# DJNing/articulated-object-nerf

Hardware: AMD Instinct MI355X
Metric: rays/sec at 640×480×(64c+128f) samples; PSNR vs reference (higher is better)
Workload: dtype f16x3 (fp16 hi/lo split MFMA, fp32 accumulate)

## Files before the change

### articulated-object-nerf_amd/aonerf/_lib.py

```python
import ctypes
import os

import torch

_HERE = os.path.dirname(os.path.abspath(__file__))
LIB_PATH = os.path.join(os.path.dirname(_HERE), "lib", "libaonerf.so")

c_i64, c_int, c_float, c_size, vp = ctypes.c_int64, ctypes.c_int, ctypes.c_float, ctypes.c_size_t, ctypes.c_void_p

PREC = {"fp32": 0, "f16x3": 1}
PREC_F16X3_TRAIN = 4
PREC_BF16 = 2
ACT_NONE, ACT_VANILLA, ACT_ARTIC = 0, 1, 2
OPACITY = {None: 0, "mse": 1, "ce": 2, "autorf": 3}


class AonMlpParams(ctypes.Structure):
    _fields_ = [("pts_w", vp * 8), ("pts_b", vp * 8), ("density_w", vp), ("density_b", vp),
                ("bottleneck_w", vp), ("bottleneck_b", vp), ("views_w", vp), ("views_b", vp),
                ("rgb_w", vp), ("rgb_b", vp), ("w_rows", c_i64 * 12), ("w_cols", c_i64 * 12),
                ("b_len", c_i64 * 12)]


class AonMlpArtParams(ctypes.Structure):
# ... 113 lines not shown
    "aon_sample_along_rays": (c_int, [vp, vp, c_i64, c_int, vp, vp, vp, vp, vp, vp]),
    "aon_pos_enc": (c_int, [vp, c_i64, c_int, c_int, vp, vp]),
    "aon_sample_rays": (c_int, [vp, vp, c_int, c_i64, c_int, c_int, c_float, vp, c_i64, c_int,
                                c_float, vp, vp, vp, vp, vp]),
    "aon_cast_rays": (c_int, [vp, vp, vp, c_i64, c_int, vp, c_i64, vp, c_int, c_int, vp, vp]),
    "aon_cast_rays_tiled": (c_int, [vp, vp, vp, c_i64, c_int, c_int, c_int, c_int, vp, vp]),
    "aon_sample_pdf": (c_int, [vp, c_i64, vp, c_i64, c_i64, c_int, c_int, vp, c_i64, vp, c_int,
                               vp, vp, vp, vp, vp]),
    "aon_composite_march": (c_int, [vp, vp, vp, c_i64, c_int, c_int, c_int, vp, c_i64, c_int, vp,
                                    vp, vp, vp, vp, vp]),
    "aon_mlp_packed_bytes": (c_size, [c_int]),
    "aon_mlp_read_status": (c_int, [vp, c_size, ctypes.POINTER(ctypes.c_uint32), vp]),
    "aon_mlp_pack": (c_int, [ctypes.POINTER(AonMlpParams), c_int, vp, vp]),
    "aon_mlp_fwd": (c_int, [vp, c_int, vp, vp, vp, vp, c_i64, c_int, c_int, vp, vp]),
    "aon_mlp_fwd_encoded": (c_int, [vp, c_int, vp, vp, c_i64, c_int, c_int, vp, vp]),
    "aon_mlp_fwd_train": (c_int, [vp, vp, vp, vp, vp, c_i64, c_int, vp, vp, vp, vp, vp, vp, vp]),
    "aon_mlp_fwd_train_bf16": (c_int, [vp, vp, vp, vp, vp, c_i64, c_int, vp, vp, vp, vp, vp, vp,
                                       vp, vp]),
    "aon_mlp_bwd_pack_bf16": (c_int, [ctypes.POINTER(AonMlpParams), vp, vp]),
    "aon_mlp_bwd_bf16": (c_int, [vp, vp, vp, c_i64, vp, vp, vp, vp, vp]),
    "aon_relu_masks": (c_int, [vp, c_i64, c_int, vp, vp]),
    "aon_absmax": (c_int, [vp, c_i64, vp, vp]),
    "aon_mlp_bwd_packed_bytes": (c_size, []),
    "aon_mlp_bwd_pack": (c_int, [ctypes.POINTER(AonMlpParams), vp, vp]),
    "aon_mlp_bwd": (c_int, [vp, vp, vp, c_i64, vp, vp, vp, vp, vp]),
    "aon_mlp_art_packed_bytes": (c_size, []),
    "aon_mlp_art_pack": (c_int, [ctypes.POINTER(AonMlpArtParams), vp, vp]),
    "aon_mlp_art_fwd": (c_int, [vp, vp, vp, vp, vp, c_i64, c_int, c_int, vp, vp]),
    "aon_mlp_art_fwd_points": (c_int, [vp, vp, vp, c_i64, c_int, c_int, vp, vp]),
    "aon_mlp_art_bwd_packed_bytes": (c_size, []),
# ... 195 lines not shown
```

### articulated-object-nerf_amd/aonerf/model.py

```python
import warnings

import torch
import torch.nn as nn
import torch.nn.init as init

from . import _lib as L
from . import helper
from .numerics import resolve as _resolve_numerics

_DEFAULT_GEOMETRY = dict(min_deg_point=0, max_deg_point=10, deg_view=4, netdepth=8, netwidth=256,
                         netdepth_condition=1, netwidth_condition=128, skip_layer=4, input_ch=3,
                         input_ch_view=3, num_rgb_channels=3, num_density_channels=1)


class NeRFMLP(nn.Module):

    def __init__(self, min_deg_point, max_deg_point, deg_view, netdepth: int = 8,
                 netwidth: int = 256, netdepth_condition: int = 1, netwidth_condition: int = 128,
                 skip_layer: int = 4, input_ch: int = 3, input_ch_view: int = 3,
                 num_rgb_channels: int = 3, num_density_channels: int = 1,
                 precision: str = "f16x3"):
        super().__init__()
        self.min_deg_point, self.max_deg_point, self.deg_view = min_deg_point, max_deg_point, deg_view
        self.netdepth, self.netwidth, self.skip_layer = netdepth, netwidth, skip_layer
# ... 45 lines not shown
        params = [p for m in self._layers() for p in (m.weight, m.bias)]
        L.require_gpu(*params)
        key = (self.precision,) + tuple((p.data_ptr(), p._version) for p in params)
        if key != self._packed_key:
            params = [L.contig(p.detach()) for p in params]
            prm = L.mlp_params(zip(params[0::2], params[1::2]))
            prec = L.PREC[self.precision]
            nbytes = L.lib().aon_mlp_packed_bytes(prec)
            if nbytes == 0:
                raise NotImplementedError(f"precision {self.precision!r} is not built yet")
            buf = torch.empty(nbytes // 4, dtype=torch.float32, device=params[0].device)
            L.call("aon_mlp_pack", L.ctypes.byref(prm), prec, L.ptr(buf), L.stream(buf.device))
            self._packed, self._packed_key = buf, key
        return self._packed

    def forward_rays(self, rays_o, rays_d, viewdirs, t_vals, act=L.ACT_NONE):
        L.require_gpu(rays_o, rays_d, viewdirs, t_vals)
        B, S = t_vals.shape
        raw = torch.empty((B * S, 4), device=t_vals.device)
        L.call("aon_mlp_fwd", L.ptr(self.packed_weights()), L.PREC[self.precision],
               L.ptr(L.contig(rays_o)), L.ptr(L.contig(rays_d)), L.ptr(L.contig(viewdirs)),
               L.ptr(L.contig(t_vals)), B, S, act, L.ptr(raw), L.stream(t_vals.device))
        return raw

    def forward(self, x, condition):
        L.require_gpu(x, condition)
        B, S, C = x.shape
        if C != 63 or tuple(condition.shape) != (B, 27):
            raise ValueError("NeRFMLP.forward expects x (B, S, 63) and condition (B, 27)")
        raw = torch.empty((B * S, 4), device=x.device)
        L.call("aon_mlp_fwd_encoded", L.ptr(self.packed_weights()), L.PREC[self.precision],
               L.ptr(L.contig(x)), L.ptr(L.contig(condition)), B, S, L.ACT_NONE, L.ptr(raw),
               L.stream(x.device))
        raw = raw.view(B, S, 4)
        return raw[..., :3], raw[..., 3:]


# ... 68 lines not shown
        self.fused_march, self.range_check = bool(fused_march), bool(range_check)
        self.num_levels, self.min_deg_point, self.max_deg_point = num_levels, min_deg_point, max_deg_point
        self.deg_view, self.num_coarse_samples, self.num_fine_samples = deg_view, num_coarse_samples, num_fine_samples
        self.use_viewdirs, self.noise_std, self.lindisp = use_viewdirs, noise_std, lindisp
        self.coarse_mlp = NeRFMLP(min_deg_point, max_deg_point, deg_view, precision=precision)
        self.fine_mlp = NeRFMLP(min_deg_point, max_deg_point, deg_view, precision=precision)

    def set_precision(self, precision):
        for m in (self.coarse_mlp, self.fine_mlp):
            if precision not in L.PREC:
                raise ValueError(precision)
            m.precision = precision
        return self

    def forward(self, rays, randomized, white_bkgd, near, far, *, u_coarse=None, u_fine=None,
                return_weights=False, return_intermediates=False, timers=None):
        o, d, v = rays["rays_o"], rays["rays_d"], rays["viewdirs"]
        L.require_gpu(o, d, v)
        o, d, v = L.contig(o), L.contig(d), L.contig(v)
        training = torch.is_grad_enabled() and any(p.requires_grad for p in self.parameters())
        B = o.shape[0]
        dev = o.device
        rng = torch.cuda.get_rng_state(dev) if randomized and not training else None
        ret = []
        t_vals = weights = t_next = None
        token, joined = None, {}
        cfg = self.train_numerics
        if training:
            from . import train
            if cfg.overlap_dweight and cfg.fused_backward and timers is None:
                token = train.JoinToken()
                ps = [p for m in (self.coarse_mlp, self.fine_mlp) for l in m._layers()
                      for p in (l.weight, l.bias)]
                joined = dict(zip(map(id, ps), train.Join.apply(token, *ps)))
        for level in range(2):
            with torch.no_grad():
                t_vals = t_next if t_next is not None else self._level_t(
# ... 9 lines not shown
                params = [joined.get(id(p), p) for p in params]
                comp, acc, depth, weights = RenderLevel.apply(o, d, v, t_vals, bool(white_bkgd),
                                                              noise, token, cfg, timers, *params)
                out = (comp, acc, depth, weights) if return_weights else (comp, acc, depth)
                if return_intermediates:
                    out = out + (dict(t_vals=t_vals, weights=weights),)
                ret.append(out)
                continue
            keep_w = level == 0 or return_weights or return_intermediates
            march = level == 0 and march_ok(S, self.num_fine_samples, self.fused_march)
            if march:
                keep_w = return_weights or return_intermediates
            with torch.no_grad():
                out, weights, t_next = self._render_level_fused(
                    mlp, o, d, v, t_vals, randomized, white_bkgd, level, timers, keep_w,
                    march_u=(lambda: fine_uniforms(B, self.num_fine_samples, randomized, dev,
                                                   u_fine)) if march else None)
            if not return_weights:
                out = out[:3] + out[4:]
            if not return_intermediates:
                out = out[:4] if return_weights else out[:3]
            ret.append(out)
        if (not training and self.range_check and self.coarse_mlp.precision.startswith("f16x3")
                and not torch.cuda.is_current_stream_capturing()
                and L.range_overflow([self.coarse_mlp._packed, self.fine_mlp._packed])):
            warnings.warn("NeRF: an MLP activation exceeded the fp16x3 range; re-rendered with "
                          "precision='fp32'", RuntimeWarning)
            prec = self.coarse_mlp.precision
            self.set_precision("fp32")
            if rng is not None:
                torch.cuda.set_rng_state(rng, dev)
            try:
                return self.forward(rays, randomized, white_bkgd, near, far, u_coarse=u_coarse,
                                    u_fine=u_fine, return_weights=return_weights,
                                    return_intermediates=return_intermediates, timers=timers)
            finally:
                self.set_precision(prec)
        return ret

    def _level_t(self, level, o, d, t_prev, w_prev, randomized, near, far, u_coarse, u_fine):
        return level_t_vals(level, o, d, t_prev, w_prev, randomized, near, far,
                            self.num_coarse_samples, self.num_fine_samples, self.lindisp,
                            u_coarse, u_fine)

    def _render_level_fused(self, mlp, o, d, v, t_vals, randomized, white_bkgd, level, timers,
                            keep_weights=True, march_u=None):
        B, S = t_vals.shape
        dev = o.device
        noisy = self.noise_std > 0 and randomized
        ev = _events(timers)
        raw = mlp.forward_rays(o, d, v, t_vals, act=L.ACT_NONE if noisy else L.ACT_VANILLA)
        _record(timers, ev, f"mlp{level}", B * S)
        if noisy:
            raw[:, 3] += torch.rand_like(raw[:, 3]) * self.noise_std
        act = L.ACT_VANILLA if noisy else L.ACT_NONE
        t_next = None
        ev = _events(timers)
        if march_u is not None:
            u, u_stride = march_u()
            (comp, acc, depth, weights), t_next = composite_march(
                raw, t_vals, d, white_bkgd, act, u, u_stride, self.num_fine_samples, keep_weights)
            _record(timers, ev, f"march{level}", B * S)
        else:
            comp = torch.empty((B, 3), device=dev)
            acc = torch.empty((B,), device=dev)
            weights = torch.empty((B, S), device=dev) if keep_weights else None
# ... 7 lines not shown
```

### articulated-object-nerf_amd/aonerf/render.py

```python
import math
from collections import defaultdict

import numpy as np
import torch

from . import interface
from .ray_utils import frame_rays

DEFAULT_CHUNK = 1 << 21


def _chunks(B, chunk):
    chunk = max(int(chunk or DEFAULT_CHUNK), 1)
    for i in range(0, B, chunk):
        yield i, min(i + chunk, B)


@torch.no_grad()
def render_rays(model, batch, chunk, white_bkgd, near, far):
    B = batch["rays_o"].shape[0]
    ret = defaultdict(list)
    for i, j in _chunks(B, chunk):
        sub = {k: batch[k][i:j] for k in ("rays_o", "rays_d", "viewdirs")}
        fine = model(sub, False, white_bkgd, near, far)[1]
        ret["comp_rgb"].append(fine[0])
        ret["acc"].append(fine[1])
        ret["depth"].append(fine[2])
    out = {k: torch.cat(v, 0) for k, v in ret.items()}
    if "target" in batch:
        out["psnr"] = interface.psnr_legacy(out["comp_rgb"], batch["target"]).mean()
    return out


@torch.no_grad()
def render_rays_test(model, batch, chunk, white_bkgd, near, far):
    out = render_rays(model, {k: v for k, v in batch.items() if k != "target"}, chunk, white_bkgd,
                      near, far)
    test_output = {"rgb": out["comp_rgb"]}
    for k in ("target", "instance_mask"):
        if k in batch:
            test_output[k] = batch[k]
    return test_output


@torch.no_grad()
def render_frame(model, c2w, H, W, focal, near=2.0, far=6.0, white_bkgd=True, p0=0, n=None,
                 chunk=None, timers=None):
    n = H * W - p0 if n is None else n
    rays = frame_rays(c2w, H, W, focal, p0, n)
    out = torch.empty((n, 5), device=rays["rays_o"].device)
    for i, j in _chunks(n, chunk):
        sub = {k: v[i:j] for k, v in rays.items()}
        fine = model(sub, False, white_bkgd, near, far, timers=timers)[1]
        out[i:j, 0:3] = fine[0]
        out[i:j, 3] = fine[2]
        out[i:j, 4] = fine[1]
    return out


def create_spheric_poses(radius=4.0, n=40, phi=-30.0):

    def trans_t(t):
        return np.array([[1, 0, 0, 0], [0, 1, 0, 0], [0, 0, 1, t], [0, 0, 0, 1]], np.float32)

    def rot_phi(p):
        c, s = np.cos(p), np.sin(p)
        return np.array([[1, 0, 0, 0], [0, c, -s, 0], [0, s, c, 0], [0, 0, 0, 1]], np.float32)

# ... 17 lines not shown
```

### articulated-object-nerf_amd/csrc/mlp.hip

```cpp
#include "aon_common.hpp"
#include "mlp_layout.hpp"
#include "mlp_pipe.hpp"
#include "param_check.hpp"

namespace aon {
namespace mlp {

constexpr int kWaves = 8;
constexpr int kThreads = 64 * kWaves;
constexpr int kRowsPerWave = 16;
constexpr int kRowsPerBlock = kRowsPerWave * kWaves;

__device__ __forceinline__ f4 mfma(float a, float b, f4 c) {
  return __builtin_amdgcn_mfma_f32_16x16x4f32(a, b, c, 0, 0, 0);
}

template <int LAYER, int NA, int NB, int NACC>
__device__ __forceinline__ void gemm(Pipe<kThreads>& p, const f4 (&xa)[NA], const f4 (&xb)[NB],
                                     f4 (&acc)[NACC]) {
  constexpr LayerDesc d = kLayers[LAYER];
  constexpr int U = d.u;
  static_assert(U % 4 == 0 && U <= NACC && d.ka <= NA && d.kb <= NB, "layer/array mismatch");
#pragma unroll
  for (int t = 0; t < d.ka + d.kb; ++t) {
// ... 293 lines not shown
}

extern "C" int aon_mlp_fwd(const void* packed, int precision, const float* rays_o,
                           const float* rays_d, const float* viewdirs, const float* t, int64_t B,
                           int S, int act, float* raw, aon_stream_t stream) {
  AON_REQUIRE(viewdirs && t, "null pointer");
  return mlp_launch(0, packed, precision, rays_o, rays_d, viewdirs, t, B, S, act, raw, stream);
}

extern "C" int aon_mlp_fwd_encoded(const void* packed, int precision, const float* x,
                                   const float* condition, int64_t B, int S, int act,
                                   float* raw, aon_stream_t stream) {
  return mlp_launch(1, packed, precision, x, condition, nullptr, nullptr, B, S, act, raw, stream);
}

extern "C" int aon_mlp_fwd_train(const void* packed, const float* rays_o, const float* rays_d,
                                 const float* viewdirs, const float* t, int64_t B, int S,
                                 const float* noise, float* h, float* bot, float* hv, float* raw,
                                 uint32_t* masks, aon_stream_t stream) {
  AON_REQUIRE(packed && rays_o && rays_d && viewdirs && t && h && bot && hv && raw && masks,
              "null pointer");
  AON_REQUIRE(aligned16(masks), "masks must be 16-byte aligned");
  AON_REQUIRE(B >= 0 && S >= 1, "bad shape");
  AON_REQUIRE(aligned16(packed) && aligned16(raw) && aligned16(h) && aligned16(bot) && aligned16(hv),
              "packed / output buffers must be 16-byte aligned");
  const int64_t N = B * S;
  if (N == 0) return 0;
  AON_REQUIRE((N + 127) / 128 < (1ll << 31), "too many rows");
  const TrainStore ts{h, bot, hv, noise, reinterpret_cast<uint2*>(masks)};
  return launch_f16x3(2, 1, packed, rays_o, rays_d, viewdirs, t, B, S, AON_ACT_NONE, raw,
// ... 24 lines not shown
```

### articulated-object-nerf_amd/csrc/mlp_f16x3.hip

```cpp
#include "mlp_f16x3_core.hpp"

namespace aon {
namespace mlp {

#ifndef AON_STASH_REGS
#define AON_STASH_REGS 0
#endif

#ifndef AON_STAGGER
#define AON_STAGGER 0
#endif

template <bool BF>
__host__ __device__ constexpr int stash_per() { return BF ? 3 : 6; }
template <bool BF>
__device__ __forceinline__ int enc_slot(int c, int k, int lo) { return BF ? 3 * c + k : 6 * c + 2 * k + lo; }
template <bool BF>
__device__ __forceinline__ int venc_slot(int c, int lo) { return BF ? 3 * c + 2 : 6 * c + 4 + lo; }

template <typename Net, int NCOL, bool STORE, typename T, typename FP>
__device__ __forceinline__ void vanilla_layers(FP& fp, Frag<2, NCOL>& enc, Frag<1, NCOL>& venc,
                                               Frag<8, NCOL>& x, Frag<8, NCOL>& y, f4* stash,
                                               float* bias_s, int g, int wave,
                                               const int64_t (&rows)[NCOL], int64_t N, int act,
                                               float* __restrict__ raw, const TrainStore& ts) {
  constexpr bool BF = std::is_same<T, __bf16>::value;
  fp.start();
#if AON_PRIO_HALF
  if (wave >= GeomH<NCOL>::kWaves / 2) __builtin_amdgcn_s_setprio(AON_PRIO_HALF);
#endif
  lds_float* bias_l = opaque_lds(bias_s + 4 * g);

  Frag<1, NCOL> none;
  using SP = StorePick<STORE, NCOL, T>;
  T* const th = reinterpret_cast<T*>(ts.h);
  T* const tbot = reinterpret_cast<T*>(ts.bot);
  T* const thv = reinterpret_cast<T*>(ts.hv);
  const int64_t hs = act_rows(N) * 256;
  const int64_t ms = act_rows(N) * 4;
  layer_h<Net, L0, true>(fp, none, enc, x, bias_l, g, SP::make(th, 256, rows, N, g, ts.masks));
  layer_h<Net, L1, true>(fp, x, none, y, bias_l, g, SP::make(th + 1 * hs, 256, rows, N, g, ts.masks + 1 * ms));
  layer_h<Net, L2, true>(fp, y, none, x, bias_l, g, SP::make(th + 2 * hs, 256, rows, N, g, ts.masks + 2 * ms));
  layer_h<Net, L3, true>(fp, x, none, y, bias_l, g, SP::make(th + 3 * hs, 256, rows, N, g, ts.masks + 3 * ms));
  layer_h<Net, L4, true>(fp, y, none, x, bias_l, g, SP::make(th + 4 * hs, 256, rows, N, g, ts.masks + 4 * ms));
#pragma unroll
  for (int c = 0; c < NCOL && !AON_STASH_REGS; ++c)
#pragma unroll
    for (int k = 0; k < 2; ++k) {
      enc.hi[k][c] = __builtin_bit_cast(h8, stash[64 * enc_slot<BF>(c, k, 0)]);
      if (!BF) enc.lo[k][c] = __builtin_bit_cast(h8, stash[64 * enc_slot<BF>(c, k, 1)]);
    }
  layer_h<Net, L5, true>(fp, x, enc, y, bias_l, g, SP::make(th + 5 * hs, 256, rows, N, g, ts.masks + 5 * ms));
  layer_h<Net, L6, true>(fp, y, none, x, bias_l, g, SP::make(th + 6 * hs, 256, rows, N, g, ts.masks + 6 * ms));
  layer_h<Net, L7, true>(fp, x, none, y, bias_l, g, SP::make(th + 7 * hs, 256, rows, N, g, ts.masks + 7 * ms));
  f4 dens[NCOL], rgb[NCOL];
  head_h<Net, LDEN>(fp, y, dens, bias_l, g);
  constexpr bool FOLD = std::is_same<Net, NetVanillaFoldH>::value;
  static_assert(!FOLD || !STORE, "the training forwards keep the bottleneck activation");
  if constexpr (!FOLD)
    layer_h<Net, LBOT, false>(fp, y, none, x, bias_l, g, SP::make(tbot, 256, rows, N, g));
#pragma unroll
  for (int c = 0; c < NCOL && !AON_STASH_REGS; ++c) {
    venc.hi[0][c] = __builtin_bit_cast(h8, stash[64 * venc_slot<BF>(c, 0)]);
    if (!BF) venc.lo[0][c] = __builtin_bit_cast(h8, stash[64 * venc_slot<BF>(c, 1)]);
  }
  if constexpr (FOLD) {
    layer_h<Net, LF_VIEW, true>(fp, y, venc, x, bias_l, g);
    head_h<Net, LF_RGB>(fp, x, rgb, bias_l, g);
  } else {
    layer_h<Net, LVIEW, true>(fp, x, venc, y, bias_l, g, SP::make(thv, 128, rows, N, g, ts.masks + 8 * ms));
    head_h<Net, LRGB>(fp, y, rgb, bias_l, g);
  }

  if (g == 0) {
#pragma unroll
    for (int c = 0; c < NCOL; ++c) {
      if (rows[c] < N) {
        const float s = AON_F16X3_V2 ? 1.0f : 1.0f / kActScale;
        float sig = dens[c][0] * s;
        if (STORE && ts.noise) sig = __fadd_rn(sig, ts.noise[rows[c]]);
        const f4 o = {act_rgb(rgb[c][0] * s, act), act_rgb(rgb[c][1] * s, act),
                      act_rgb(rgb[c][2] * s, act), act_sigma(sig, act)};
#ifdef AON_ABL_NO_RAW_STORE
        if (__builtin_isnan(o[0] + o[1] + o[2] + o[3]))
#endif
        *reinterpret_cast<f4*>(raw + 4 * rows[c]) = o;
      }
    }
  }
}

template <int MODE, int NCOL, bool STORE = false, bool BF = false, typename Net = NetVanillaH>
__global__ __launch_bounds__((GeomH<NCOL, BF>::kThreads), (GeomH<NCOL, BF>::kWavesPerSimd)) void k_mlp_fwd_f16x3(
    const f4* __restrict__ wstream, const float* __restrict__ bias_g, const float* __restrict__ in0,
    const float* __restrict__ in1, const float* __restrict__ in2, const float* __restrict__ in3,
    int64_t B, int S, int act, float* __restrict__ raw, TrainStore ts = {}) {
  using G = GeomH<NCOL, BF>;
  constexpr int kPer = stash_per<BF>() * NCOL;
  constexpr int kStash = AON_STASH_REGS ? 0 : G::kWaves * 64 * kPer;
  static_assert((kLdsWeights + Net::kBiasFloats / 4 + kStash) * 16 <= 160 * 1024, "LDS");
  __shared__ f4 smem[kLdsWeights + Net::kBiasFloats / 4 + kStash];
  float* bias_s = reinterpret_cast<float*>(smem + kLdsWeights);
  f4* stash = smem + kLdsWeights + Net::kBiasFloats / 4 + (threadIdx.x >> 6) * 64 * kPer +
              (threadIdx.x & 63);

  const int tid = threadIdx.x, lane = tid & 63, wave = tid >> 6;
  const int g = lane >> 4, j = lane & 15;
  const int64_t N = B * S;

  WeightPipeP<Net, G::kThreads, BF> p;
  p.wbuf = smem;
  p.src = wstream;
  p.tid = tid;
  p.lane = lane;
  p.start();
  for (int i = tid; i < Net::kBiasFloats; i += G::kThreads) bias_s[i] = bias_g[i];

  Frag<2, NCOL> enc;
  Frag<1, NCOL> venc;
  int64_t rows[NCOL];
#pragma unroll
  for (int c = 0; c < NCOL; ++c) {
    const int64_t row = (int64_t)blockIdx.x * G::kRowsPerBlock + wave * G::kRowsPerWave + 16 * c + j;
    rows[c] = row;
    const int64_t rr = row < N ? row : N - 1;
    const int64_t ray = rr / S;
    float ev[2][8], vv[8];
    if (MODE == 0) {
      const float* ro = in0 + 3 * ray;
      const float* rd = in1 + 3 * ray;
      const float* vd = in2 + 3 * ray;
      const float tt = in3[rr];
      const float x0 = __fadd_rn(ro[0], __fmul_rn(tt, rd[0]));
      const float x1 = __fadd_rn(ro[1], __fmul_rn(tt, rd[1]));
      const float x2 = __fadd_rn(ro[2], __fmul_rn(tt, rd[2]));
      const float v0 = vd[0], v1 = vd[1], v2 = vd[2];
      auto encode = [&](auto fast) {
#pragma unroll
        for (int k = 0; k < 2; ++k)
#pragma unroll
          for (int e = 0; e < 8; ++e)
          {
            ev[k][e] = pos_enc_feature_fast(x0, x1, x2, 32 * k + 8 * g + e, 0, 10, fast.value);
            __builtin_amdgcn_sched_barrier(0);
          }
#pragma unroll
        for (int e = 0; e < 8; ++e) {
          vv[e] = pos_enc_feature_fast(v0, v1, v2, 8 * g + e, 0, 4, fast.value);
          __builtin_amdgcn_sched_barrier(0);
        }
      };
      if (pos_enc_fast_ok(x0, x1, x2, 10) && pos_enc_fast_ok(v0, v1, v2, 4))
        encode(std::true_type{});
      else
        encode(std::false_type{});
    } else {
      const float* x = in0 + rr * 63;
      const float* cd = in1 + ray * 27;
#pragma unroll
      for (int k = 0; k < 2; ++k)
#pragma unroll
        for (int e = 0; e < 8; ++e) {
          const int f = 32 * k + 8 * g + e;
          ev[k][e] = f < 63 ? x[f] : 0.f;
        }
#pragma unroll
      for (int e = 0; e < 8; ++e) {
        const int f = 8 * g + e;
        vv[e] = f < 27 ? cd[f] : 0.f;
      }
    }
    if (STORE && BF && ts.enc_bf && keep_row(rows[c], N)) store_enc_bf(ts.enc_bf, rows[c], g, ev);
#pragma unroll
    for (int k = 0; k < 2; ++k) {
#pragma unroll
      for (int e = 0; e < 8; ++e) ev[k][e] *= act_scale<BF>();
      split8<BF>(ev[k], enc.hi[k][c], enc.lo[k][c], enc.ovf);
    }
#pragma unroll
    for (int e = 0; e < 8; ++e) vv[e] *= act_scale<BF>();
    split8<BF>(vv, venc.hi[0][c], venc.lo[0][c], venc.ovf);
  }

#pragma unroll
  for (int c = 0; c < NCOL && !AON_STASH_REGS; ++c) {
#pragma unroll
    for (int k = 0; k < 2; ++k) {
      stash[64 * enc_slot<BF>(c, k, 0)] = __builtin_bit_cast(f4, enc.hi[k][c]);
      if (!BF) stash[64 * enc_slot<BF>(c, k, 1)] = __builtin_bit_cast(f4, enc.lo[k][c]);
    }
    stash[64 * venc_slot<BF>(c, 0)] = __builtin_bit_cast(f4, venc.hi[0][c]);
    if (!BF) stash[64 * venc_slot<BF>(c, 1)] = __builtin_bit_cast(f4, venc.lo[0][c]);
  }

  Frag<8, NCOL> x, y;
  using WP = WeightPipeP<Net, G::kThreads, BF>;
  using T = typename std::conditional<BF, __bf16, float>::type;
  if (AON_STAGGER && NCOL == 1 && !STORE && __builtin_amdgcn_readfirstlane(wave) >= G::kWaves / 2) {
    FragPipe<WP, AON_PREFETCH, 4, BF> fp(p);
    vanilla_layers<Net, NCOL, STORE, T>(fp, enc, venc, x, y, stash, bias_s, g, wave, rows, N, act, raw, ts);
  } else {
    FragPipe<WP, AON_PREFETCH, 0, BF> fp(p);
    vanilla_layers<Net, NCOL, STORE, T>(fp, enc, venc, x, y, stash, bias_s, g, wave, rows, N, act, raw, ts);
  }
  range_report(bias_g + Net::kBiasFloats, ovf_of(x) | ovf_of(y) | enc.ovf | venc.ovf);
}

__global__ void k_pack_h(PackArgsH a, float* __restrict__ out_f) {
  const int64_t nhalf = (int64_t)a.stream_blocks * 512;
  _Float16* out = reinterpret_cast<_Float16*>(out_f);
  float* bias_out = out_f + (int64_t)a.stream_blocks * 256;
  const int64_t total = nhalf + a.bias_floats;
  const LayerDesc& last = a.layers[a.n_layers - 1];
  const int used_blocks = last.blk0 + (last.ka + last.kb) * last.u * 2;
  const StreamMap map{a.bf16, a.mx_lo, a.mx_hi};
  if (a.bf16 == 1 && !a.f16w && blockIdx.x == 0 && threadIdx.x < kStatusBytes / 4)
    reinterpret_cast<uint32_t*>(bias_out + a.bias_floats)[threadIdx.x] = 0u;
  for (int64_t e = blockIdx.x * (int64_t)blockDim.x + threadIdx.x; e < total;
       e += (int64_t)gridDim.x * blockDim.x) {
    if (e < nhalf) {
// ... 149 lines not shown
                         static_cast<int>((N + GB::kRowsPerBlock - 1) / GB::kRowsPerBlock),
                         GB::kThreads, 0, stream, ws, bias, a0, a1, a2, a3, B, S, act, raw, *ts);
    } else
      hipLaunchKernelGGL((k_mlp_fwd_f16x3<0, 1, true>), grid, GeomH<1>::kThreads, 0, stream, ws,
                         bias, a0, a1, a2, a3, B, S, act, raw, *ts);
    return launch_status("aon_mlp_fwd_train");
  }
  if (mode == 0 && ncol == 1) AON_LAUNCH_H(0, 1);
  else if (mode == 0) AON_LAUNCH_H(0, 2);
  else if (ncol == 1) AON_LAUNCH_H(1, 1);
  else AON_LAUNCH_H(1, 2);
#undef AON_LAUNCH_H
  return launch_status("aon_mlp_fwd");
}

}
}
```

### articulated-object-nerf_amd/csrc/mlp_layout.hpp

```cpp
#pragma once

namespace aon {
namespace mlp {

struct LayerDesc {
  int ka, kb;
  int u;
  int len_a, len_b;
  int out_real;
  int blk0;
  int bias0;
};

enum { L0 = 0, L1, L2, L3, L4, L5, L6, L7, LDEN, LBOT, LVIEW, LRGB, kNumLayers };

constexpr int kChunk = 16;

constexpr LayerDesc kLayers[kNumLayers] = {
    {4, 0, 16, 63, 0, 256, 0, 0},
    {16, 0, 16, 256, 0, 256, 64, 256},
    {16, 0, 16, 256, 0, 256, 320, 512},
    {16, 0, 16, 256, 0, 256, 576, 768},
    {16, 0, 16, 256, 0, 256, 832, 1024},
    {16, 4, 16, 256, 63, 256, 1088, 1280},
// ... 188 lines not shown
static_assert(NetVanillaFoldH::ok(), "inconsistent folded vanilla fp16x3 layout");
constexpr bool layout_fold_ok() {
  for (int i = 0; i < kNumLayersFold; ++i) {
    const LayerDesc& f = kLayersHFold[i];
    const LayerDesc& h = kLayersH[i < LBOT ? i : i + 1];
    if (f.ka != h.ka || f.kb != h.kb || f.u != h.u || f.len_a != h.len_a || f.len_b != h.len_b ||
        f.out_real != h.out_real)
      return false;
    if (i < LBOT && (f.blk0 != h.blk0 || f.bias0 != h.bias0)) return false;
  }
  const LayerDesc& b = kLayersH[LBOT];
  return kLayersHFold[LF_VIEW].len_a == b.out_real && kBlocksFold == kBlocks - b.ka * b.u * 2 &&
         kBiasFloatsFold == kBiasFloats - b.u * 16;
}
static_assert(layout_fold_ok(), "folded layout must be kLayersH without the bottleneck");
static_assert(NetArtH::ok(), "inconsistent articulated fp16x3 layout");
static_assert(NetBwdH::ok(), "inconsistent backward-chain fp16x3 layout");
static_assert(NetArtBwdH::ok(), "inconsistent articulated backward-chain fp16x3 layout");

struct PackArgs {
  const float* w[kNumLayers];
  const float* b[kNumLayers];
  LayerDesc layers[kNumLayers];
};

constexpr int kMaxLayersH = 24;
struct PackArgsH {
  const float* w[kMaxLayersH];
  const float* w2[kMaxLayersH];
  const float* b[kMaxLayersH];
// ... 65 lines not shown
  float* hv;
  float* enc;
  float* xyz;
  const float* noise;
  uint2* masks;
  __bf16* enc_bf;
};

int pack_f16x3(const PackArgs& a, void* packed, hipStream_t stream, bool bf16 = false,
               bool fold = false);
int pack_h(PackArgsH a, void* packed, hipStream_t stream);
int absmax(const float* x, int64_t n, uint32_t* out, hipStream_t stream);
int launch_f16x3(int mode, int ncol, const void* packed, const float* a0, const float* a1,
                 const float* a2, const float* a3, int64_t B, int S, int act, float* raw,
                 hipStream_t stream, const TrainStore* ts = nullptr);
#ifndef AON_DATAFLOW_WS_BUILD
#define AON_DATAFLOW_WS_BUILD 0
#endif
int launch_ws_f16x3(const void* packed, const float* a0, const float* a1, const float* a2,
                    const float* a3, int64_t B, int S, int act, float* raw, hipStream_t stream);
int launch_art_ws_f16x3(const void* packed, const float* a0, const float* a1, const float* a2,
                        const float* a3, int64_t B, int S, int act, float* raw, hipStream_t stream);

}
}
```

### include/aonerf.h

```cpp
#ifndef AONERF_H
#define AONERF_H

#include <stddef.h>
#include <stdint.h>

#ifdef __cplusplus
extern "C" {
#endif

typedef void* aon_stream_t;

#define AON_ABI_VERSION 13

#define AON_PREC_FP32 0
#define AON_PREC_F16X3 1
#define AON_PREC_F16X3_TRAIN 4
#define AON_PREC_BF16 2

#define AON_ACT_NONE 0
#define AON_ACT_VANILLA 1
#define AON_ACT_ARTIC 2

int aon_abi_version(void);
const char* aon_last_error(void);
// ... 53 lines not shown
size_t aon_mlp_packed_bytes(int precision);
int aon_mlp_pack(const aon_mlp_params* params, int precision, void* packed,
                 aon_stream_t stream);

int aon_mlp_read_status(const void* packed, size_t packed_bytes, uint32_t* status,
                        aon_stream_t stream);

int aon_mlp_fwd(const void* packed, int precision, const float* rays_o, const float* rays_d,
                const float* viewdirs, const float* t, int64_t B, int S, int act, float* out,
                aon_stream_t stream);


int aon_mlp_fwd_encoded(const void* packed, int precision, const float* x,
                        const float* condition, int64_t B, int S, int act, float* out,
                        aon_stream_t stream);

int aon_mlp_fwd_train(const void* packed, const float* rays_o, const float* rays_d,
                      const float* viewdirs, const float* t, int64_t B, int S, const float* noise,
                      float* h, float* bot, float* hv, float* raw, uint32_t* masks,
                      aon_stream_t stream);

int aon_mlp_fwd_train_bf16(const void* packed, const float* rays_o, const float* rays_d,
                           const float* viewdirs, const float* t, int64_t B, int S,
                           const float* noise, uint16_t* h, uint16_t* bot, uint16_t* hv,
                           float* raw, uint32_t* masks, uint16_t* enc, aon_stream_t stream);

int aon_relu_masks(const float* h, int64_t N, int width, uint32_t* masks, aon_stream_t stream);

int aon_absmax(const float* x, int64_t n, uint32_t* out, aon_stream_t stream);

// ... 171 lines not shown
```

Baseline: 1.653 million.

## Skip coarse-level RGB head in render path and precompute view encoding per ray

Adds a density-only MLP kernel that streams only the prefix of the folded weight stream up to the density head, and uses it for the coarse level when only fine outputs are requested. The fine level uses a new MODE 2 kernel that takes a per-ray precomputed view-direction encoding instead of recomputing it per sample. The render entry points now pass fine_only=True. The coarse RGB is discarded anyway, so this is meant to cut the view and RGB layers and the smaller LDS stash from the coarse pass. The cost is extra kernel variants and a per-ray pos_enc launch.

Measured after the change: 1.717 million, median of 6. 1.04x the previous value.

```diff
diff --git a/articulated-object-nerf_amd/aonerf/_lib.py b/articulated-object-nerf_amd/aonerf/_lib.py
--- a/articulated-object-nerf_amd/aonerf/_lib.py
+++ b/articulated-object-nerf_amd/aonerf/_lib.py
@@ -151,6 +151,8 @@
     "aon_mlp_pack": (c_int, [ctypes.POINTER(AonMlpParams), c_int, vp, vp]),
     "aon_mlp_fwd": (c_int, [vp, c_int, vp, vp, vp, vp, c_i64, c_int, c_int, vp, vp]),
     "aon_mlp_fwd_encoded": (c_int, [vp, c_int, vp, vp, c_i64, c_int, c_int, vp, vp]),
+    "aon_mlp_fwd_sigma": (c_int, [vp, c_int, vp, vp, vp, c_i64, c_int, c_int, vp, vp]),
+    "aon_mlp_fwd_cond": (c_int, [vp, c_int, vp, vp, vp, vp, c_i64, c_int, c_int, vp, vp]),
     "aon_mlp_fwd_train": (c_int, [vp, vp, vp, vp, vp, c_i64, c_int, vp, vp, vp, vp, vp, vp, vp]),
     "aon_mlp_fwd_train_bf16": (c_int, [vp, vp, vp, vp, vp, c_i64, c_int, vp, vp, vp, vp, vp, vp,
                                        vp, vp]),
diff --git a/articulated-object-nerf_amd/aonerf/model.py b/articulated-object-nerf_amd/aonerf/model.py
--- a/articulated-object-nerf_amd/aonerf/model.py
+++ b/articulated-object-nerf_amd/aonerf/model.py
@@ -83,13 +83,29 @@
             self._packed, self._packed_key = buf, key
         return self._packed
 
-    def forward_rays(self, rays_o, rays_d, viewdirs, t_vals, act=L.ACT_NONE):
-        L.require_gpu(rays_o, rays_d, viewdirs, t_vals)
+    def forward_rays(self, rays_o, rays_d, viewdirs, t_vals, act=L.ACT_NONE, cond=None):
+        L.require_gpu(rays_o, rays_d, viewdirs, t_vals, cond)
         B, S = t_vals.shape
         raw = torch.empty((B * S, 4), device=t_vals.device)
+        if cond is not None:
+            if tuple(cond.shape) != (B, 27):
+                raise ValueError("forward_rays expects cond (B, 27)")
+            L.call("aon_mlp_fwd_cond", L.ptr(self.packed_weights()), L.PREC[self.precision],
+                   L.ptr(L.contig(rays_o)), L.ptr(L.contig(rays_d)), L.ptr(L.contig(cond)),
+                   L.ptr(L.contig(t_vals)), B, S, act, L.ptr(raw), L.stream(t_vals.device))
+            return raw
         L.call("aon_mlp_fwd", L.ptr(self.packed_weights()), L.PREC[self.precision],
                L.ptr(L.contig(rays_o)), L.ptr(L.contig(rays_d)), L.ptr(L.contig(viewdirs)),
                L.ptr(L.contig(t_vals)), B, S, act, L.ptr(raw), L.stream(t_vals.device))
+        return raw
+
+    def forward_sigma(self, rays_o, rays_d, t_vals, act=L.ACT_NONE):
+        L.require_gpu(rays_o, rays_d, t_vals)
+        B, S = t_vals.shape
+        raw = torch.empty((B * S, 4), device=t_vals.device)
+        L.call("aon_mlp_fwd_sigma", L.ptr(self.packed_weights()), L.PREC[self.precision],
+               L.ptr(L.contig(rays_o)), L.ptr(L.contig(rays_d)), L.ptr(L.contig(t_vals)), B, S, act,
+               L.ptr(raw), L.stream(t_vals.device))
         return raw
 
     def forward(self, x, condition):
@@ -188,13 +204,16 @@
         return self
 
     def forward(self, rays, randomized, white_bkgd, near, far, *, u_coarse=None, u_fine=None,
-                return_weights=False, return_intermediates=False, timers=None):
+                return_weights=False, return_intermediates=False, timers=None, fine_only=False):
         o, d, v = rays["rays_o"], rays["rays_d"], rays["viewdirs"]
         L.require_gpu(o, d, v)
         o, d, v = L.contig(o), L.contig(d), L.contig(v)
         training = torch.is_grad_enabled() and any(p.requires_grad for p in self.parameters())
         B = o.shape[0]
         dev = o.device
+        fine_only = bool(fine_only) and not (training or return_weights or return_intermediates)
+        two_pass = fine_only and self.coarse_mlp.precision == self.fine_mlp.precision == "f16x3"
+        cond = helper.pos_enc(v, 0, self.deg_view) if two_pass else None
         rng = torch.cuda.get_rng_state(dev) if randomized and not training else None
         ret = []
         t_vals = weights = t_next = None
@@ -234,13 +253,14 @@
             with torch.no_grad():
                 out, weights, t_next = self._render_level_fused(
                     mlp, o, d, v, t_vals, randomized, white_bkgd, level, timers, keep_w,
+                    sigma_only=two_pass and level == 0, cond=cond if level == 1 else None,
                     march_u=(lambda: fine_uniforms(B, self.num_fine_samples, randomized, dev,
                                                    u_fine)) if march else None)
             if not return_weights:
                 out = out[:3] + out[4:]
             if not return_intermediates:
                 out = out[:4] if return_weights else out[:3]
-            ret.append(out)
+            ret.append(None if fine_only and level == 0 else out)
         if (not training and self.range_check and self.coarse_mlp.precision.startswith("f16x3")
                 and not torch.cuda.is_current_stream_capturing()
                 and L.range_overflow([self.coarse_mlp._packed, self.fine_mlp._packed])):
@@ -253,7 +273,8 @@
             try:
                 return self.forward(rays, randomized, white_bkgd, near, far, u_coarse=u_coarse,
                                     u_fine=u_fine, return_weights=return_weights,
-                                    return_intermediates=return_intermediates, timers=timers)
+                                    return_intermediates=return_intermediates, timers=timers,
+                                    fine_only=fine_only)
             finally:
                 self.set_precision(prec)
         return ret
@@ -264,12 +285,16 @@
                             u_coarse, u_fine)
 
     def _render_level_fused(self, mlp, o, d, v, t_vals, randomized, white_bkgd, level, timers,
-                            keep_weights=True, march_u=None):
+                            keep_weights=True, march_u=None, sigma_only=False, cond=None):
         B, S = t_vals.shape
         dev = o.device
         noisy = self.noise_std > 0 and randomized
         ev = _events(timers)
-        raw = mlp.forward_rays(o, d, v, t_vals, act=L.ACT_NONE if noisy else L.ACT_VANILLA)
+        act = L.ACT_NONE if noisy else L.ACT_VANILLA
+        if sigma_only:
+            raw = mlp.forward_sigma(o, d, t_vals, act=act)
+        else:
+            raw = mlp.forward_rays(o, d, v, t_vals, act=act, cond=cond)
         _record(timers, ev, f"mlp{level}", B * S)
         if noisy:
             raw[:, 3] += torch.rand_like(raw[:, 3]) * self.noise_std
diff --git a/articulated-object-nerf_amd/aonerf/render.py b/articulated-object-nerf_amd/aonerf/render.py
--- a/articulated-object-nerf_amd/aonerf/render.py
+++ b/articulated-object-nerf_amd/aonerf/render.py
@@ -22,7 +22,7 @@
     ret = defaultdict(list)
     for i, j in _chunks(B, chunk):
         sub = {k: batch[k][i:j] for k in ("rays_o", "rays_d", "viewdirs")}
-        fine = model(sub, False, white_bkgd, near, far)[1]
+        fine = model(sub, False, white_bkgd, near, far, fine_only=True)[1]
         ret["comp_rgb"].append(fine[0])
         ret["acc"].append(fine[1])
         ret["depth"].append(fine[2])
@@ -51,7 +51,7 @@
     out = torch.empty((n, 5), device=rays["rays_o"].device)
     for i, j in _chunks(n, chunk):
         sub = {k: v[i:j] for k, v in rays.items()}
-        fine = model(sub, False, white_bkgd, near, far, timers=timers)[1]
+        fine = model(sub, False, white_bkgd, near, far, timers=timers, fine_only=True)[1]
         out[i:j, 0:3] = fine[0]
         out[i:j, 3] = fine[2]
         out[i:j, 4] = fine[1]
diff --git a/articulated-object-nerf_amd/csrc/mlp.hip b/articulated-object-nerf_amd/csrc/mlp.hip
--- a/articulated-object-nerf_amd/csrc/mlp.hip
+++ b/articulated-object-nerf_amd/csrc/mlp.hip
@@ -331,6 +331,42 @@
   return mlp_launch(1, packed, precision, x, condition, nullptr, nullptr, B, S, act, raw, stream);
 }
 
+static int two_pass_check(const void* packed, int precision, const float* rays_o,
+                          const float* rays_d, const float* t, int64_t B, int S, int act,
+                          const float* raw) {
+  AON_REQUIRE(packed && raw && rays_o && rays_d && t, "null pointer");
+  AON_REQUIRE(precision != AON_PREC_F16X3_TRAIN,
+              "AON_PREC_F16X3_TRAIN is the training forward's stream (aon_mlp_fwd_train): render "
+              "with an AON_PREC_F16X3 pack");
+  AON_REQUIRE(precision != AON_PREC_FP32,
+              "AON_PREC_FP32 has no two-pass kernels: render a fp32 pack with aon_mlp_fwd");
+  AON_REQUIRE(precision == AON_PREC_F16X3,
+              "unsupported precision (AON_PREC_BF16 is the training forward's: aon_mlp_fwd_train_bf16)");
+  AON_REQUIRE(B >= 0 && S >= 1, "bad shape");
+  AON_REQUIRE(act >= AON_ACT_NONE && act <= AON_ACT_ARTIC, "bad activation");
+  AON_REQUIRE(aligned16(packed) && aligned16(raw), "packed / raw must be 16-byte aligned");
+  if (B * S == 0) return 1;
+  AON_REQUIRE((B * S + 127) / 128 < (1ll << 31), "too many rows");
+  return 0;
+}
+
+extern "C" int aon_mlp_fwd_sigma(const void* packed, int precision, const float* rays_o,
+                                 const float* rays_d, const float* t, int64_t B, int S, int act,
+                                 float* raw, aon_stream_t stream) {
+  const int c = two_pass_check(packed, precision, rays_o, rays_d, t, B, S, act, raw);
+  if (c) return c < 0 ? c : 0;
+  return launch_f16x3_sigma(packed, rays_o, rays_d, t, B, S, act, raw, (hipStream_t)stream);
+}
+
+extern "C" int aon_mlp_fwd_cond(const void* packed, int precision, const float* rays_o,
+                                const float* rays_d, const float* cond, const float* t, int64_t B,
+                                int S, int act, float* raw, aon_stream_t stream) {
+  AON_REQUIRE(cond, "null pointer");
+  const int c = two_pass_check(packed, precision, rays_o, rays_d, t, B, S, act, raw);
+  if (c) return c < 0 ? c : 0;
+  return launch_f16x3_cond(packed, rays_o, rays_d, cond, t, B, S, act, raw, (hipStream_t)stream);
+}
+
 extern "C" int aon_mlp_fwd_train(const void* packed, const float* rays_o, const float* rays_d,
                                  const float* viewdirs, const float* t, int64_t B, int S,
                                  const float* noise, float* h, float* bot, float* hv, float* raw,
diff --git a/articulated-object-nerf_amd/csrc/mlp_f16x3.hip b/articulated-object-nerf_amd/csrc/mlp_f16x3.hip
--- a/articulated-object-nerf_amd/csrc/mlp_f16x3.hip
+++ b/articulated-object-nerf_amd/csrc/mlp_f16x3.hip
@@ -11,12 +11,20 @@
 #define AON_STAGGER 0
 #endif
 
-template <bool BF>
-__host__ __device__ constexpr int stash_per() { return BF ? 3 : 6; }
-template <bool BF>
-__device__ __forceinline__ int enc_slot(int c, int k, int lo) { return BF ? 3 * c + k : 6 * c + 2 * k + lo; }
+template <bool BF, bool SIG = false>
+__host__ __device__ constexpr int stash_per() { return BF ? 3 : (SIG ? 4 : 6); }
+template <bool BF, bool SIG = false>
+__device__ __forceinline__ int enc_slot(int c, int k, int lo) {
+  return BF ? 3 * c + k : stash_per<BF, SIG>() * c + 2 * k + lo;
+}
 template <bool BF>
 __device__ __forceinline__ int venc_slot(int c, int lo) { return BF ? 3 * c + 2 : 6 * c + 4 + lo; }
+
+template <typename Net>
+constexpr bool kSigmaOnly = std::is_same<Net, NetVanillaSigmaH>::value;
+static_assert(kStreamBlocksSigma % kChunkH == 0 &&
+                  (kBlocksSigma - 1) / kChunkH == kStreamBlocksSigma / kChunkH - 1,
+              "density-only stream: whole ring chunks, none unused");
 
 template <typename Net, int NCOL, bool STORE, typename T, typename FP>
 __device__ __forceinline__ void vanilla_layers(FP& fp, Frag<2, NCOL>& enc, Frag<1, NCOL>& venc,
@@ -25,6 +33,8 @@
                                                const int64_t (&rows)[NCOL], int64_t N, int act,
                                                float* __restrict__ raw, const TrainStore& ts) {
   constexpr bool BF = std::is_same<T, __bf16>::value;
+  constexpr bool SIG = kSigmaOnly<Net>;
+  static_assert(!SIG || (!STORE && !BF), "the density-only pass is a render pass");
   fp.start();
 #if AON_PRIO_HALF
   if (wave >= GeomH<NCOL>::kWaves / 2) __builtin_amdgcn_s_setprio(AON_PRIO_HALF);
@@ -47,8 +57,8 @@
   for (int c = 0; c < NCOL && !AON_STASH_REGS; ++c)
 #pragma unroll
     for (int k = 0; k < 2; ++k) {
-      enc.hi[k][c] = __builtin_bit_cast(h8, stash[64 * enc_slot<BF>(c, k, 0)]);
-      if (!BF) enc.lo[k][c] = __builtin_bit_cast(h8, stash[64 * enc_slot<BF>(c, k, 1)]);
+      enc.hi[k][c] = __builtin_bit_cast(h8, stash[64 * enc_slot<BF, SIG>(c, k, 0)]);
+      if (!BF) enc.lo[k][c] = __builtin_bit_cast(h8, stash[64 * enc_slot<BF, SIG>(c, k, 1)]);
     }
   layer_h<Net, L5, true>(fp, x, enc, y, bias_l, g, SP::make(th + 5 * hs, 256, rows, N, g, ts.masks + 5 * ms));
   layer_h<Net, L6, true>(fp, y, none, x, bias_l, g, SP::make(th + 6 * hs, 256, rows, N, g, ts.masks + 6 * ms));
@@ -57,19 +67,21 @@
   head_h<Net, LDEN>(fp, y, dens, bias_l, g);
   constexpr bool FOLD = std::is_same<Net, NetVanillaFoldH>::value;
   static_assert(!FOLD || !STORE, "the training forwards keep the bottleneck activation");
-  if constexpr (!FOLD)
-    layer_h<Net, LBOT, false>(fp, y, none, x, bias_l, g, SP::make(tbot, 256, rows, N, g));
-#pragma unroll
-  for (int c = 0; c < NCOL && !AON_STASH_REGS; ++c) {
-    venc.hi[0][c] = __builtin_bit_cast(h8, stash[64 * venc_slot<BF>(c, 0)]);
-    if (!BF) venc.lo[0][c] = __builtin_bit_cast(h8, stash[64 * venc_slot<BF>(c, 1)]);
-  }
-  if constexpr (FOLD) {
-    layer_h<Net, LF_VIEW, true>(fp, y, venc, x, bias_l, g);
-    head_h<Net, LF_RGB>(fp, x, rgb, bias_l, g);
-  } else {
-    layer_h<Net, LVIEW, true>(fp, x, venc, y, bias_l, g, SP::make(thv, 128, rows, N, g, ts.masks + 8 * ms));
-    head_h<Net, LRGB>(fp, y, rgb, bias_l, g);
+  if constexpr (!SIG) {
+    if constexpr (!FOLD)
+      layer_h<Net, LBOT, false>(fp, y, none, x, bias_l, g, SP::make(tbot, 256, rows, N, g));
+#pragma unroll
+    for (int c = 0; c < NCOL && !AON_STASH_REGS; ++c) {
+      venc.hi[0][c] = __builtin_bit_cast(h8, stash[64 * venc_slot<BF>(c, 0)]);
+      if (!BF) venc.lo[0][c] = __builtin_bit_cast(h8, stash[64 * venc_slot<BF>(c, 1)]);
+    }
+    if constexpr (FOLD) {
+      layer_h<Net, LF_VIEW, true>(fp, y, venc, x, bias_l, g);
+      head_h<Net, LF_RGB>(fp, x, rgb, bias_l, g);
+    } else {
+      layer_h<Net, LVIEW, true>(fp, x, venc, y, bias_l, g, SP::make(thv, 128, rows, N, g, ts.masks + 8 * ms));
+      head_h<Net, LRGB>(fp, y, rgb, bias_l, g);
+    }
   }
 
   if (g == 0) {
@@ -79,8 +91,12 @@
         const float s = AON_F16X3_V2 ? 1.0f : 1.0f / kActScale;
         float sig = dens[c][0] * s;
         if (STORE && ts.noise) sig = __fadd_rn(sig, ts.noise[rows[c]]);
-        const f4 o = {act_rgb(rgb[c][0] * s, act), act_rgb(rgb[c][1] * s, act),
-                      act_rgb(rgb[c][2] * s, act), act_sigma(sig, act)};
+        f4 o = {0.0f, 0.0f, 0.0f, act_sigma(sig, act)};
+        if constexpr (!SIG) {
+          o[0] = act_rgb(rgb[c][0] * s, act);
+          o[1] = act_rgb(rgb[c][1] * s, act);
+          o[2] = act_rgb(rgb[c][2] * s, act);
+        }
 #ifdef AON_ABL_NO_RAW_STORE
         if (__builtin_isnan(o[0] + o[1] + o[2] + o[3]))
 #endif
@@ -96,7 +112,9 @@
     const float* __restrict__ in1, const float* __restrict__ in2, const float* __restrict__ in3,
     int64_t B, int S, int act, float* __restrict__ raw, TrainStore ts = {}) {
   using G = GeomH<NCOL, BF>;
-  constexpr int kPer = stash_per<BF>() * NCOL;
+  constexpr bool SIG = kSigmaOnly<Net>;
+  static_assert(!SIG || MODE == 0, "the density-only pass takes MODE 0 inputs");
+  constexpr int kPer = stash_per<BF, SIG>() * NCOL;
   constexpr int kStash = AON_STASH_REGS ? 0 : G::kWaves * 64 * kPer;
   static_assert((kLdsWeights + Net::kBiasFloats / 4 + kStash) * 16 <= 160 * 1024, "LDS");
   __shared__ f4 smem[kLdsWeights + Net::kBiasFloats / 4 + kStash];
@@ -126,7 +144,7 @@
     const int64_t rr = row < N ? row : N - 1;
     const int64_t ray = rr / S;
     float ev[2][8], vv[8];
-    if (MODE == 0) {
+    if constexpr (MODE == 0 && !SIG) {
       const float* ro = in0 + 3 * ray;
       const float* rd = in1 + 3 * ray;
       const float* vd = in2 + 3 * ray;
@@ -154,6 +172,35 @@
         encode(std::true_type{});
       else
         encode(std::false_type{});
+    } else if constexpr (MODE == 0 || MODE == 2) {
+      const float* ro = in0 + 3 * ray;
+      const float* rd = in1 + 3 * ray;
+      const float tt = in3[rr];
+      const float x0 = __fadd_rn(ro[0], __fmul_rn(tt, rd[0]));
+      const float x1 = __fadd_rn(ro[1], __fmul_rn(tt, rd[1]));
+      const float x2 = __fadd_rn(ro[2], __fmul_rn(tt, rd[2]));
+      auto encode = [&](auto fast) {
+#pragma unroll
+        for (int k = 0; k < 2; ++k)
+#pragma unroll
+          for (int e = 0; e < 8; ++e)
+          {
+            ev[k][e] = pos_enc_feature_fast(x0, x1, x2, 32 * k + 8 * g + e, 0, 10, fast.value);
+            __builtin_amdgcn_sched_barrier(0);
+          }
+      };
+      if (pos_enc_fast_ok(x0, x1, x2, 10))
+        encode(std::true_type{});
+      else
+        encode(std::false_type{});
+      if constexpr (MODE == 2) {
+        const float* cd = in2 + ray * 27;
+#pragma unroll
+        for (int e = 0; e < 8; ++e) {
+          const int f = 8 * g + e;
+          vv[e] = f < 27 ? cd[f] : 0.f;
+        }
+      }
     } else {
       const float* x = in0 + rr * 63;
       const float* cd = in1 + ray * 27;
@@ -177,20 +224,24 @@
       for (int e = 0; e < 8; ++e) ev[k][e] *= act_scale<BF>();
       split8<BF>(ev[k], enc.hi[k][c], enc.lo[k][c], enc.ovf);
     }
-#pragma unroll
-    for (int e = 0; e < 8; ++e) vv[e] *= act_scale<BF>();
-    split8<BF>(vv, venc.hi[0][c], venc.lo[0][c], venc.ovf);
+    if constexpr (!SIG) {
+#pragma unroll
+      for (int e = 0; e < 8; ++e) vv[e] *= act_scale<BF>();
+      split8<BF>(vv, venc.hi[0][c], venc.lo[0][c], venc.ovf);
+    }
   }
 
 #pragma unroll
   for (int c = 0; c < NCOL && !AON_STASH_REGS; ++c) {
 #pragma unroll
     for (int k = 0; k < 2; ++k) {
-      stash[64 * enc_slot<BF>(c, k, 0)] = __builtin_bit_cast(f4, enc.hi[k][c]);
-      if (!BF) stash[64 * enc_slot<BF>(c, k, 1)] = __builtin_bit_cast(f4, enc.lo[k][c]);
-    }
-    stash[64 * venc_slot<BF>(c, 0)] = __builtin_bit_cast(f4, venc.hi[0][c]);
-    if (!BF) stash[64 * venc_slot<BF>(c, 1)] = __builtin_bit_cast(f4, venc.lo[0][c]);
+      stash[64 * enc_slot<BF, SIG>(c, k, 0)] = __builtin_bit_cast(f4, enc.hi[k][c]);
+      if (!BF) stash[64 * enc_slot<BF, SIG>(c, k, 1)] = __builtin_bit_cast(f4, enc.lo[k][c]);
+    }
+    if constexpr (!SIG) {
+      stash[64 * venc_slot<BF>(c, 0)] = __builtin_bit_cast(f4, venc.hi[0][c]);
+      if (!BF) stash[64 * venc_slot<BF>(c, 1)] = __builtin_bit_cast(f4, venc.lo[0][c]);
+    }
   }
 
   Frag<8, NCOL> x, y;
@@ -203,7 +254,8 @@
     FragPipe<WP, AON_PREFETCH, 0, BF> fp(p);
     vanilla_layers<Net, NCOL, STORE, T>(fp, enc, venc, x, y, stash, bias_s, g, wave, rows, N, act, raw, ts);
   }
-  range_report(bias_g + Net::kBiasFloats, ovf_of(x) | ovf_of(y) | enc.ovf | venc.ovf);
+  constexpr int kStatusAt = SIG ? NetVanillaFoldH::kBiasFloats : Net::kBiasFloats;
+  range_report(bias_g + kStatusAt, ovf_of(x) | ovf_of(y) | enc.ovf | venc.ovf);
 }
 
 __global__ void k_pack_h(PackArgsH a, float* __restrict__ out_f) {
@@ -383,5 +435,33 @@
   return launch_status("aon_mlp_fwd");
 }
 
-}
-}
+static const float* fold_bias(const void* packed) {
+  return reinterpret_cast<const float*>(static_cast<const char*>(packed) +
+                                        NetVanillaFoldH::kStreamBytes);
+}
+
+int launch_f16x3_sigma(const void* packed, const float* rays_o, const float* rays_d,
+                       const float* t, int64_t B, int S, int act, float* raw, hipStream_t stream) {
+  using G = GeomH<1>;
+  const int64_t N = B * S;
+  hipLaunchKernelGGL((k_mlp_fwd_f16x3<0, 1, false, false, NetVanillaSigmaH>),
+                     static_cast<int>((N + G::kRowsPerBlock - 1) / G::kRowsPerBlock), G::kThreads, 0,
+                     stream, static_cast<const f4*>(packed), fold_bias(packed), rays_o, rays_d,
+                     static_cast<const float*>(nullptr), t, B, S, act, raw);
+  return launch_status("aon_mlp_fwd_sigma");
+}
+
+int launch_f16x3_cond(const void* packed, const float* rays_o, const float* rays_d,
+                      const float* cond, const float* t, int64_t B, int S, int act, float* raw,
+                      hipStream_t stream) {
+  using G = GeomH<1>;
+  const int64_t N = B * S;
+  hipLaunchKernelGGL((k_mlp_fwd_f16x3<2, 1, false, false, NetVanillaFoldH>),
+                     static_cast<int>((N + G::kRowsPerBlock - 1) / G::kRowsPerBlock), G::kThreads, 0,
+                     stream, static_cast<const f4*>(packed), fold_bias(packed), rays_o, rays_d, cond,
+                     t, B, S, act, raw);
+  return launch_status("aon_mlp_fwd_cond");
+}
+
+}
+}
diff --git a/articulated-object-nerf_amd/csrc/mlp_layout.hpp b/articulated-object-nerf_amd/csrc/mlp_layout.hpp
--- a/articulated-object-nerf_amd/csrc/mlp_layout.hpp
+++ b/articulated-object-nerf_amd/csrc/mlp_layout.hpp
@@ -226,6 +226,32 @@
          kBiasFloatsFold == kBiasFloats - b.u * 16;
 }
 static_assert(layout_fold_ok(), "folded layout must be kLayersH without the bottleneck");
+
+constexpr int kNumLayersSigma = LDEN + 1;
+constexpr int kBlocksSigma = 1936;
+constexpr int kStreamBlocksSigma = (kBlocksSigma + 31) / 32 * 32;
+constexpr int kBiasFloatsSigma = 2064;
+struct NetVanillaSigmaH
+    : NetH<kLayersHFold, kNumLayersSigma, kBlocksSigma, kStreamBlocksSigma, kBiasFloatsSigma> {};
+constexpr bool layout_sigma_ok() {
+  int blk = 0, bias = 0;
+  for (int i = 0; i < kNumLayersSigma; ++i) {
+    const LayerDesc s = NetVanillaSigmaH::layer(i);
+    const LayerDesc& f = kLayersHFold[i];
+    if (s.ka != f.ka || s.kb != f.kb || s.u != f.u || s.len_a != f.len_a || s.len_b != f.len_b ||
+        s.out_real != f.out_real || s.blk0 != f.blk0 || s.bias0 != f.bias0)
+      return false;
+    if (f.blk0 != blk || f.bias0 != bias) return false;
+    blk += (f.ka + f.kb) * f.u * 2;
+    bias += f.u * 16;
+  }
+  return blk == kBlocksSigma && bias == kBiasFloatsSigma &&
+         kLayersHFold[LF_VIEW].blk0 == kBlocksSigma &&
+         kLayersHFold[LF_VIEW].bias0 == kBiasFloatsSigma &&
+         kBiasFloatsSigma % 4 == 0 && kStreamBlocksSigma >= kBlocksSigma &&
+         kStreamBlocksSigma <= kStreamBlocksFold;
+}
+static_assert(layout_sigma_ok(), "the density-only pass must be a prefix of the folded stream");
 static_assert(NetArtH::ok(), "inconsistent articulated fp16x3 layout");
 static_assert(NetBwdH::ok(), "inconsistent backward-chain fp16x3 layout");
 static_assert(NetArtBwdH::ok(), "inconsistent articulated backward-chain fp16x3 layout");
@@ -321,6 +347,11 @@
 int launch_f16x3(int mode, int ncol, const void* packed, const float* a0, const float* a1,
                  const float* a2, const float* a3, int64_t B, int S, int act, float* raw,
                  hipStream_t stream, const TrainStore* ts = nullptr);
+int launch_f16x3_sigma(const void* packed, const float* rays_o, const float* rays_d,
+                       const float* t, int64_t B, int S, int act, float* raw, hipStream_t stream);
+int launch_f16x3_cond(const void* packed, const float* rays_o, const float* rays_d,
+                      const float* cond, const float* t, int64_t B, int S, int act, float* raw,
+                      hipStream_t stream);
 #ifndef AON_DATAFLOW_WS_BUILD
 #define AON_DATAFLOW_WS_BUILD 0
 #endif
diff --git a/include/aonerf.h b/include/aonerf.h
--- a/include/aonerf.h
+++ b/include/aonerf.h
@@ -91,6 +91,13 @@
 int aon_mlp_fwd_encoded(const void* packed, int precision, const float* x,
                         const float* condition, int64_t B, int S, int act, float* out,
                         aon_stream_t stream);
+
+int aon_mlp_fwd_sigma(const void* packed, int precision, const float* rays_o, const float* rays_d,
+                      const float* t, int64_t B, int S, int act, float* out, aon_stream_t stream);
+
+int aon_mlp_fwd_cond(const void* packed, int precision, const float* rays_o, const float* rays_d,
+                     const float* cond, const float* t, int64_t B, int S, int act, float* out,
+                     aon_stream_t stream);
 
 int aon_mlp_fwd_train(const void* packed, const float* rays_o, const float* rays_d,
                       const float* viewdirs, const float* t, int64_t B, int S, const float* noise,
```
